# PasaLab/marlin

Hardware: AMD Instinct MI355X
Metric: dense C=AxB TFLOP/s (fp64) (higher is better)
Workload: dtype f64; 1 GPU; dgemm_20000x20000x20000_f64; m=20000, k=20000, n=20000, parallelism=single_gpu

## Files before the change

### marlin_amd/csrc/kernels.hip

```cpp

#include <hip/hip_runtime.h>
#include <stdint.h>
#include <stdlib.h>

#include <type_traits>

#include "../../include/marlin_gpu.h"
#include "gemm_group_plan.h"

typedef double v4d __attribute__((ext_vector_type(4)));
typedef float v4f __attribute__((ext_vector_type(4)));

#define DEVFN __device__ __forceinline__

DEVFN v4d mfma_16x16x4(double a, double b, v4d c) {
    return __builtin_amdgcn_mfma_f64_16x16x4f64(a, b, c, 0, 0, 0);
}
DEVFN v4f mfma_16x16x4(float a, float b, v4f c) {
    return __builtin_amdgcn_mfma_f32_16x16x4f32(a, b, c, 0, 0, 0);
}

template <typename T> struct acc_t;
template <> struct acc_t<double> { using type = v4d; };
template <> struct acc_t<float>  { using type = v4f; };

DEVFN void glds16(const void* g, void* lds) {
    __builtin_amdgcn_global_load_lds(
        (const __attribute__((address_space(1))) uint32_t*)g,
        (__attribute__((address_space(3))) uint32_t*)lds, 16, 0, 0);
}

DEVFN int32_t sload(const int32_t* p) {
    return __builtin_amdgcn_readfirstlane(*p);
}
DEVFN int64_t sload(const int64_t* p) {
    const int64_t v = *p;
    const uint32_t lo = __builtin_amdgcn_readfirstlane((uint32_t)v);
    const uint32_t hi = __builtin_amdgcn_readfirstlane((uint32_t)(v >> 32));
    return (int64_t)(((uint64_t)hi << 32) | lo);
}
DEVFN const void* sload_ptr(const void* const* p) {
    return (const void*)(uintptr_t)sload((const int64_t*)p);
}
DEVFN void* sload_ptr(void* const* p) {
    return (void*)(uintptr_t)sload((const int64_t*)p);
}

#define STAGE_FN DEVFN
#include "gemm_stage.h"

template <class S, typename T>
DEVFN void issue_pieces(const char* origin, int64_t ld, T* lds, int img,
                        int wid, int lane) {
    #pragma unroll
    for (int i = 0; i < S::PIECES; i++) {
        const stage_piece p = S::piece(wid, i, lane);
        glds16(origin + S::uni_bytes(p, ld) + S::lane_bytes(p, ld),
               &lds[img + p.lds]);
    }
}

DEVFN void block_remap(int id, int nbn, int nbm, int band, int& bm, int& bn) {
    int abands = band < 0 ? -band : band;
    int per_band = nbm * abands;
    int b0 = id / per_band;
    int w = id - b0 * per_band;
    int first_bn = b0 * abands;
    int bw = min(abands, nbn - first_bn);
    if (band < 0) {
        bn = first_bn + w / nbm;
        bm = w % nbm;
    } else {
        int sh = 8 * bw;
        int t = w / sh, l = w - t * sh;
        bm = t * 8 + l / bw;
        bn = first_bn + l % bw;
    }
}

enum { EPI_STORE = 0, EPI_TN_ADD = 1 };

template <typename T, int BETA, int BK, int BM, int WM, int WN, int PIPE,
          int TA = 0, int TB = 0, int EPI = EPI_STORE, int GRP = 0>
__launch_bounds__(WM * WN * 64, 2)
__global__ void gemm_mfma_kernel(int64_t M, int64_t N, int64_t K,
                                 const T* __restrict__ A_, int64_t lda_,
                                 const T* __restrict__ B_, int64_t ldb_,
                                 T* __restrict__ C_, int64_t ldc_,
                                 int nbm_ ,
                                 int band_ ,
                                 int phase_mask ,
                                 const T* __restrict__ addC ,
                                 const mx_group_entry* __restrict__ grp) {
    constexpr int BN = 128;
    constexpr int NWAVES = WM * WN;
    constexpr int MT = (BM / WM) / 16;
    constexpr int NT = (BN / WN) / 16;
    using ACC = typename acc_t<T>::type;
    using SA = std::conditional_t<TA != 0, stage_k<T, BM, BK, NWAVES>,
                                           stage_r<T, BM, BK, NWAVES>>;
    using SB = std::conditional_t<TB != 0, stage_r<T, BN, BK, NWAVES>,
                                           stage_k<T, BN, BK, NWAVES>>;
    constexpr int P = SA::PIECES + SB::PIECES;

    const T* __restrict__ A = A_;
    const T* __restrict__ B = B_;
    T* __restrict__ C = C_;
    int64_t lda = lda_, ldb = ldb_, ldc = ldc_;
    int nbm = nbm_, nbn = (int)(N / BN), band = band_;
    int grp_ntiles = 0;
    int id = blockIdx.x;
    if constexpr (GRP != 0) {
        static_assert(BK == 16 && BM == 128 && WM == 2 && WN == 2 &&
                      EPI == EPI_STORE, "grouped: default geometry only");
        const int count = nbm_;
        const int32_t* __restrict__ tile_start = (const int32_t*)(grp + count);
        int lo = 0, hi = count - 1;
        while (lo < hi) {
            const int mid = (lo + hi + 1) >> 1;
            if (sload(&tile_start[mid]) <= id) lo = mid; else hi = mid - 1;
        }
        const mx_group_entry* __restrict__ e = grp + lo;
        A = (const T*)sload_ptr(&e->A);
        B = (const T*)sload_ptr(&e->B);
        C = (T*)sload_ptr(&e->C);
        lda = sload(&e->lda); ldb = sload(&e->ldb); ldc = sload(&e->ldc);
        grp_ntiles = sload(&e->ntiles);
        nbm = sload(&e->nbm); nbn = sload(&e->nbn); band = sload(&e->band);
        id -= sload(&tile_start[lo]);
    }
    int bn, bm;
    block_remap(id, nbn, nbm, band, bm, bn);

    const int tid = threadIdx.x;
    const int lane = tid & 63;
    const int wid = tid >> 6;
    const int wm = wid / WN, wn = wid % WN;
    const int l15 = lane & 15, l4 = lane >> 4;

    __shared__ __align__(16) T sAB[2 * BK * BM + 2 * BN * BK];
    T* As = sAB;
    T* Bs = sAB + 2 * BK * BM;

    const int64_t row0 = (int64_t)bm * BM;
    const int64_t col0 = (int64_t)bn * BN;

    constexpr bool REGMAJOR = sizeof(T) == 8;
    const int rbase = REGMAJOR ? l4 : l4 * 4;
    constexpr int rstep = REGMAJOR ? 4 : 1;
    ACC acc[MT][NT];
    if (BETA) {
        #pragma unroll
        for (int mt = 0; mt < MT; mt++)
            #pragma unroll
            for (int nt = 0; nt < NT; nt++) {
                int64_t r = row0 + wm * (MT * 16) + mt * 16 + rbase;
                int64_t cc = col0 + wn * (NT * 16) + nt * 16 + l15;
                const T* cp = C + cc * ldc + r;
                #pragma unroll
                for (int j = 0; j < 4; j++) acc[mt][nt][j] = cp[rstep * j];
            }
    } else {
        #pragma unroll
        for (int mt = 0; mt < MT; mt++)
            #pragma unroll
            for (int nt = 0; nt < NT; nt++) acc[mt][nt] = ACC{0};
    }

    const int ntiles = GRP != 0 ? grp_ntiles : (int)(K / BK);
    const int ph = (phase_mask && (id & phase_mask)) ? (ntiles >> 1) : 0;

    auto read_quad = [&](const T* At, const T* Bt, int q, T (&a)[MT],
                         T (&b)[NT]) {
        const int kk = q * 4 + l4;
        #pragma unroll
        for (int mt = 0; mt < MT; mt++)
            a[mt] = At[SA::frag(wm * (MT * 16) + mt * 16 + l15, kk)];
        #pragma unroll
        for (int nt = 0; nt < NT; nt++)
            b[nt] = Bt[SB::frag(wn * (NT * 16) + nt * 16 + l15, kk)];
    };
    auto mfma_quad = [&](const T (&a)[MT], const T (&b)[NT]) {
        #pragma unroll
        for (int mt = 0; mt < MT; mt++)
            #pragma unroll
            for (int nt = 0; nt < NT; nt++)
                acc[mt][nt] = mfma_16x16x4(a[mt], b[nt], acc[mt][nt]);
    };

    if constexpr (!PIPE) {
    auto issue_tile = [&](int kt, int buf) {
        const int64_t kbase = (int64_t)kt * BK;
        issue_pieces<SA>((const char*)(A + SA::origin_elems(lda, row0, kbase)),
                         lda, As, buf * BK * BM, wid, lane);
        issue_pieces<SB>((const char*)(B + SB::origin_elems(ldb, col0, kbase)),
                         ldb, Bs, buf * BN * BK, wid, lane);
    };
    issue_tile(ph, 0);

    for (int s = 0; s < ntiles; s++) {
        const int buf = s & 1;
        if (s + 1 < ntiles) {
            int nxt = s + 1 + ph;
            if (nxt >= ntiles) nxt -= ntiles;
            issue_tile(nxt, buf ^ 1);
            asm volatile("s_waitcnt vmcnt(%0)" :: "n"(P) : "memory");
        } else {
            asm volatile("s_waitcnt vmcnt(0)" ::: "memory");
        }
        __builtin_amdgcn_s_barrier();

        const T* At = &As[buf * BK * BM];
        const T* Bt = &Bs[buf * BN * BK];
        #pragma unroll
        for (int q = 0; q < BK / 4; q++) {
            T a[MT], b[NT];
            read_quad(At, Bt, q, a, b);
            mfma_quad(a, b);
        }
        asm volatile("s_waitcnt lgkmcnt(0)" ::: "memory");
        __builtin_amdgcn_s_barrier();
    }
    } else {
    constexpr int Q = BK / 4;
    static_assert(Q % 2 == 0, "fragment registers ping-pong per quad");
    const int swid = __builtin_amdgcn_readfirstlane(wid);
    uint32_t a_lane[SA::PIECES], b_lane[SB::PIECES];
    int64_t a_uni[SA::PIECES], b_uni[SB::PIECES];
    int a_lds[SA::PIECES], b_lds[SB::PIECES];
    #pragma unroll
    for (int i = 0; i < SA::PIECES; i++) {
        const stage_piece p = SA::piece(swid, i, lane);
        a_lane[i] = (uint32_t)SA::lane_bytes(p, lda);
        a_uni[i] = SA::uni_bytes(p, lda);
        a_lds[i] = p.lds;
    }
    #pragma unroll
    for (int i = 0; i < SB::PIECES; i++) {
        const stage_piece p = SB::piece(swid, i, lane);
        b_lane[i] = (uint32_t)SB::lane_bytes(p, ldb);
        b_uni[i] = SB::uni_bytes(p, ldb);
        b_lds[i] = p.lds;
    }

    const char* const pA0 = (const char*)(A + SA::origin_elems(lda, row0, 0));
    const char* const pB0 = (const char*)(B + SB::origin_elems(ldb, col0, 0));
    const int64_t stepA = SA::origin_elems(lda, 0, BK) * (int64_t)sizeof(T);
    const int64_t stepB = SB::origin_elems(ldb, 0, BK) * (int64_t)sizeof(T);
    const char* pA = pA0 + ph * stepA;
    const char* pB = pB0 + ph * stepB;
    int kt = ph;
    auto issue_next = [&](int buf) {
        #pragma unroll
        for (int i = 0; i < SA::PIECES; i++)
            glds16(pA + a_uni[i] + a_lane[i], &As[buf * BK * BM + a_lds[i]]);
        #pragma unroll
        for (int i = 0; i < SB::PIECES; i++)
            glds16(pB + b_uni[i] + b_lane[i], &Bs[buf * BN * BK + b_lds[i]]);
        kt++; pA += stepA; pB += stepB;
        if (kt == ntiles) { kt = 0; pA = pA0; pB = pB0; }
    };

    T fa[2][MT], fb[2][NT];
    issue_next(0);
    if (ntiles > 1) {
        issue_next(1);
        asm volatile("s_waitcnt vmcnt(%0)" :: "n"(P) : "memory");
    } else {
        asm volatile("s_waitcnt vmcnt(0)" ::: "memory");
    }
    __builtin_amdgcn_s_barrier();
    read_quad(As, Bs, 0, fa[0], fb[0]);

    auto step = [&](int s, auto ahead) {
        constexpr int AHEAD = decltype(ahead)::value;
        const int buf = s & 1;
        const T* At = &As[buf * BK * BM];
        const T* Bt = &Bs[buf * BN * BK];
        #pragma unroll
        for (int q = 0; q + 1 < Q; q++) {
            read_quad(At, Bt, q + 1, fa[(q + 1) & 1], fb[(q + 1) & 1]);
            mfma_quad(fa[q & 1], fb[q & 1]);
        }
        __builtin_amdgcn_sched_barrier(0);
        asm volatile("s_waitcnt lgkmcnt(0)" ::: "memory");
        if constexpr (AHEAD >= 1) {
            asm volatile("s_waitcnt vmcnt(0)" ::: "memory");
            __builtin_amdgcn_s_barrier();
            __builtin_amdgcn_sched_barrier(0);
            read_quad(&As[(buf ^ 1) * BK * BM], &Bs[(buf ^ 1) * BN * BK], 0,
                      fa[0], fb[0]);
            if constexpr (AHEAD >= 2) issue_next(buf);
        }
        mfma_quad(fa[1], fb[1]);
        if constexpr (AHEAD >= 1) {
            #pragma unroll
            for (int g = 0; g < MT + NT; g++) {
                __builtin_amdgcn_sched_group_barrier(0x008, 1, 0);
                __builtin_amdgcn_sched_group_barrier(0x100, 1, 0);
            }
            if constexpr (AHEAD >= 2) {
                #pragma unroll
                for (int g = 0; g < P; g++) {
                    __builtin_amdgcn_sched_group_barrier(0x008, 1, 0);
                    __builtin_amdgcn_sched_group_barrier(0x010, 1, 0);
                }
            }
        }
        __builtin_amdgcn_sched_barrier(0);
    };
    int s = 0;
    for (; s + 2 < ntiles; s++) step(s, std::integral_constant<int, 2>{});
    if (s + 1 < ntiles) { step(s, std::integral_constant<int, 1>{}); s++; }
    step(s, std::integral_constant<int, 0>{});
    }

    if constexpr (EPI == EPI_TN_ADD) {
        static_assert(std::is_same<T, float>::value && !BETA && !PIPE &&
                      BM == 128 && WM == 2 && WN == 2,
                      "fused epilogue: fp32 default geometry, two-barrier loop");
        static_assert(64 * BN == 2 * BK * BM + 2 * BN * BK,
                      "the 64x128 stage fills the k-loop buffers exactly");
        float* stage = sAB;
        v4f* stage4 = (v4f*)sAB;
        #pragma unroll
        for (int half = 0; half < 2; half++) {
            __builtin_amdgcn_s_barrier();
            if (wm == half) {
                #pragma unroll
                for (int mt = 0; mt < 4; mt++)
                    #pragma unroll
                    for (int nt = 0; nt < 4; nt++) {
                        int rloc = mt * 16 + l4 * 4;
                        int cc = wn * 64 + nt * 16 + l15;
                        #pragma unroll
                        for (int j = 0; j < 4; j++)
                            stage[(rloc + j) * BN + cc] = acc[mt][nt][j];
                    }
            }
            __builtin_amdgcn_s_barrier();
            #pragma unroll
            for (int i = 0; i < 8; i++) {
                int idx = tid + i * 256;
                int rloc = idx >> 5;
                int q = idx & 31;
                int64_t r = row0 + half * 64 + rloc;
                int64_t off = col0 + 4 * q + r * ldc;
                v4f v = stage4[rloc * (BN / 4) + q];
                if (addC) {
                    const v4f* ap = (const v4f*)(addC + off);
                    v4f av = *ap;
                    v.x += av.x; v.y += av.y; v.z += av.z; v.w += av.w;
                }
                *(v4f*)(C + off) = v;
            }
        }
    } else {
    #pragma unroll
    for (int mt = 0; mt < MT; mt++)
        #pragma unroll
        for (int nt = 0; nt < NT; nt++) {
            int64_t r = row0 + wm * (MT * 16) + mt * 16 + rbase;
            int64_t cc = col0 + wn * (NT * 16) + nt * 16 + l15;
            T* cp = C + cc * ldc + r;
            #pragma unroll
            for (int j = 0; j < 4; j++) cp[rstep * j] = acc[mt][nt][j];
        }
    }
}


__device__ __forceinline__ uint64_t splitmix64(uint64_t z) {
    z = (z ^ (z >> 30)) * 0xBF58476D1CE4E5B9ULL;
    z = (z ^ (z >> 27)) * 0x94D049BB133111EBULL;
    return z ^ (z >> 31);
}

template <typename T>
__global__ void fill_random_kernel(T* __restrict__ buf, int64_t m, int64_t n,
                                   int64_t ld, uint64_t seed) {
    int64_t i = (int64_t)blockIdx.x * blockDim.x + threadIdx.x;
    int64_t total = m * n;
    int64_t stride = (int64_t)gridDim.x * blockDim.x;
    for (; i < total; i += stride) {
        int64_t c = i / m, r = i - c * m;
        uint64_t z = splitmix64(seed + (uint64_t)(i + 1) * 0x9E3779B97F4A7C15ULL);
        buf[c * ld + r] = (T)((double)(z >> 11) * (1.0 / 9007199254740992.0));
    }
}

template <typename T>
__global__ void zero_pad_kernel(T* __restrict__ buf, int64_t rows_total,
                                int64_t cols_total, int64_t ld,
                                int64_t m, int64_t n) {
    int64_t i = (int64_t)blockIdx.x * blockDim.x + threadIdx.x;
    int64_t total = rows_total * cols_total;
    int64_t stride = (int64_t)gridDim.x * blockDim.x;
    for (; i < total; i += stride) {
        int64_t c = i / rows_total, r = i - c * rows_total;
        if (r >= m || c >= n) buf[c * ld + r] = (T)0;
    }
}


template <typename T>
__global__ void map_kernel(int op, int64_t n, const T* __restrict__ a,
                           const T* __restrict__ b, double scalar,
                           T* __restrict__ c) {
    const T s = (T)scalar;
    int64_t i = (int64_t)blockIdx.x * blockDim.x + threadIdx.x;
    int64_t stride = (int64_t)gridDim.x * blockDim.x;
    for (; i < n; i += stride) {
        T x = a[i];
        T y;
        switch (op) {
            case MX_OP_ADD:   y = x + b[i]; break;
            case MX_OP_SUB:   y = x - b[i]; break;
            case MX_OP_EMUL:  y = x * b[i]; break;
            case MX_OP_ADDS:  y = x + s; break;
            case MX_OP_SUBS:  y = x - s; break;
            case MX_OP_RSUBS: y = s - x; break;
            case MX_OP_MULS:  y = x * s; break;
            case MX_OP_DIVS:  y = x / s; break;
            default:          y = s / x; break;
        }
        c[i] = y;
    }
}

template <typename T>
__global__ void sum_stage1_kernel(int64_t n, const T* __restrict__ a,
                                  double* __restrict__ partials) {
    __shared__ double sm[256];
    double acc = 0;
    int64_t i = (int64_t)blockIdx.x * blockDim.x + threadIdx.x;
    int64_t stride = (int64_t)gridDim.x * blockDim.x;
    for (; i < n; i += stride) acc += (double)a[i];
    sm[threadIdx.x] = acc;
    __syncthreads();
    for (int w = 128; w > 0; w >>= 1) {
        if (threadIdx.x < w) sm[threadIdx.x] += sm[threadIdx.x + w];
        __syncthreads();
    }
    if (threadIdx.x == 0) partials[blockIdx.x] = sm[0];
}

__global__ void sum_stage2_kernel(int nparts, const double* __restrict__ p,
                                  double* __restrict__ out) {
    __shared__ double sm[256];
    double acc = 0;
    for (int i = threadIdx.x; i < nparts; i += 256) acc += p[i];
    sm[threadIdx.x] = acc;
    __syncthreads();
    for (int w = 128; w > 0; w >>= 1) {
        if (threadIdx.x < w) sm[threadIdx.x] += sm[threadIdx.x + w];
        __syncthreads();
    }
    if (threadIdx.x == 0) *out = sm[0];
}

template <typename T>
__global__ void transpose_kernel(int64_t m, int64_t n,
                                 const T* __restrict__ in,
                                 T* __restrict__ out) {
    __shared__ T tile[32][33];
    int64_t tm = (m + 31) / 32;
    int64_t bi = blockIdx.x % tm;
    int64_t bj = blockIdx.x / tm;
    int tx = threadIdx.x % 32, ty = threadIdx.x / 32;
    int64_t r0 = bi * 32, c0 = bj * 32;
    #pragma unroll
    for (int k = 0; k < 4; k++) {
        int64_t r = r0 + tx, c = c0 + ty + k * 8;
        if (r < m && c < n) tile[ty + k * 8][tx] = in[c * m + r];
    }
    __syncthreads();
    #pragma unroll
    for (int k = 0; k < 4; k++) {
        int64_t r = c0 + tx, c = r0 + ty + k * 8;
        if (r < n && c < m) out[c * n + r] = tile[tx][ty + k * 8];
    }
}

template <typename T>
__global__ void gemv_partial_kernel(int64_t m, int64_t n, int64_t lda,
                                    const T* __restrict__ A,
                                    const T* __restrict__ x,
                                    double* __restrict__ partial,
                                    int nchunks) {
    int64_t nrb = (m + 255) / 256;
    int64_t rb = blockIdx.x % nrb;
    int chunk = (int)(blockIdx.x / nrb);
    int64_t r = rb * 256 + threadIdx.x;
    int64_t clen = (n + nchunks - 1) / nchunks;
    int64_t c0 = chunk * clen;
    int64_t c1 = c0 + clen < n ? c0 + clen : n;
    if (r >= m) return;
    double a0 = 0, a1 = 0, a2 = 0, a3 = 0;
    int64_t j = c0;
    for (; j + 4 <= c1; j += 4) {
        a0 += (double)A[(j + 0) * lda + r] * (double)x[j + 0];
        a1 += (double)A[(j + 1) * lda + r] * (double)x[j + 1];
        a2 += (double)A[(j + 2) * lda + r] * (double)x[j + 2];
        a3 += (double)A[(j + 3) * lda + r] * (double)x[j + 3];
    }
    for (; j < c1; j++)
        a0 += (double)A[j * lda + r] * (double)x[j];
    partial[(int64_t)chunk * m + r] = ((a0 + a1) + (a2 + a3));
}

template <typename T>
__global__ void gemv_reduce_kernel(int64_t m, int nchunks,
                                   const double* __restrict__ partial,
                                   T* __restrict__ y) {
    int64_t r = (int64_t)blockIdx.x * blockDim.x + threadIdx.x;
    if (r >= m) return;
    double acc = 0;
    for (int c = 0; c < nchunks; c++) acc += partial[(int64_t)c * m + r];
    y[r] = (T)acc;
}

static mx_gemm_cfg_t g_last_gemm_cfg = {};
static int g_last_gemm_loop = 0;
static int g_last_gemm_op[2] = {0, 0};

struct gemm_call {
    int64_t M, N, K;
    const void* A; int64_t lda;
    const void* B; int64_t ldb;
    void* C; int64_t ldc;
    int band, phase_mask;
    int loopsel;
    bool pitch32;
    hipStream_t stream;
};

template <typename T, int BETA, int BK, int BM, int WM, int WN,
          int TA = 0, int TB = 0>
static void launch_gemm(const gemm_call& g) {
    const bool pipe = g.pitch32 && (g.loopsel >= 0 ? g.loopsel == 1
                                    : !(sizeof(T) == 4 && BK == 16));
    g_last_gemm_cfg = mx_gemm_cfg_t{sizeof(T) == 4, BETA, BK, BM, WM * WN,
                                    g.band, g.phase_mask};
    g_last_gemm_loop = pipe ? 1 : 0;
    g_last_gemm_op[0] = TA;
    g_last_gemm_op[1] = TB;
    auto go = [&](auto pipe_c) {
        hipLaunchKernelGGL(
            (gemm_mfma_kernel<T, BETA, BK, BM, WM, WN, decltype(pipe_c)::value,
                              TA, TB>),
            dim3((unsigned)((g.M / BM) * (g.N / 128))), dim3(WM * WN * 64),
            0, g.stream, g.M, g.N, g.K, (const T*)g.A, g.lda,
            (const T*)g.B, g.ldb, (T*)g.C, g.ldc, (int)(g.M / BM), g.band,
            g.phase_mask, (const T*)nullptr,
            (const mx_group_entry*)nullptr);
    };
    if (pipe) go(std::integral_constant<int, 1>{});
    else      go(std::integral_constant<int, 0>{});
}

static int g_last_gemm_group_problems = 0;
static int64_t g_last_gemm_group_blocks = 0;

template <typename T, int BETA, int TA, int TB>
static void launch_gemm_grouped(int count, unsigned blocks, int band0,
                                const mx_group_entry* table, int loopsel,
                                bool pitch32, hipStream_t stream) {
    const bool pipe = pitch32 && (loopsel >= 0 ? loopsel == 1
                                  : sizeof(T) != 4);
    g_last_gemm_cfg = mx_gemm_cfg_t{sizeof(T) == 4, BETA, 16, 128, 4, band0, 0};
    g_last_gemm_loop = pipe ? 1 : 0;
    g_last_gemm_op[0] = TA;
    g_last_gemm_op[1] = TB;
    g_last_gemm_group_problems = count;
    g_last_gemm_group_blocks = blocks;
    auto go = [&](auto pipe_c) {
        hipLaunchKernelGGL(
            (gemm_mfma_kernel<T, BETA, 16, 128, 2, 2, decltype(pipe_c)::value,
                              TA, TB, EPI_STORE, 1>),
            dim3(blocks), dim3(256), 0, stream, (int64_t)0, (int64_t)0,
            (int64_t)0, (const T*)nullptr, (int64_t)0, (const T*)nullptr,
            (int64_t)0, (T*)nullptr, (int64_t)0, count, 0, 0,
            (const T*)nullptr, table);
    };
    if (pipe) go(std::integral_constant<int, 1>{});
    else      go(std::integral_constant<int, 0>{});
}

extern "C" {

void mxk_gemm_remap_knobs(int* band_width, int* plain_bands) {
    static const char* bandenv = getenv("MARLIN_GEMM_BAND");
    static const char* remap = getenv("MARLIN_GEMM_REMAP");
    int bandw = bandenv ? atoi(bandenv) : 8;
    *band_width = bandw < 1 ? 8 : bandw;
    *plain_bands = remap && remap[0] == 'b';
}

void mxk_last_gemm_group(int* problems, int64_t* blocks) {
    *problems = g_last_gemm_group_problems;
    *blocks = g_last_gemm_group_blocks;
}

int mxk_gemm_grouped(int is_fp32, int beta_one, int trans_a, int trans_b,
                     const mx_group_plan* plan, void* ws, hipStream_t stream) {
    const int count = (int)plan->entries.size();
    if (count == 0) return 0;
    const size_t eb = (size_t)count * sizeof(mx_group_entry);
    if (hipMemcpyAsync(ws, plan->entries.data(), eb, hipMemcpyHostToDevice,
                       stream) != hipSuccess ||
        hipMemcpyAsync((char*)ws + eb, plan->tile_start.data(),
                       (size_t)(count + 1) * sizeof(int32_t),
                       hipMemcpyHostToDevice, stream) != hipSuccess)
        return -2;
    static const char* loopenv = getenv("MARLIN_GEMM_LOOP");
    const int loopsel = !loopenv ? -1 : loopenv[0] == 't' ? 0
                      : loopenv[0] == 'p' ? 1 : -1;
    const unsigned blocks = (unsigned)plan->blocks();
    const int band0 = plan->entries[0].band;
    const mx_group_entry* table = (const mx_group_entry*)ws;
    auto form = [&](auto t, auto beta) {
        using T = decltype(t);
        constexpr int BT = decltype(beta)::value;
        auto l = [&](auto ta, auto tb) {
            launch_gemm_grouped<T, BT, decltype(ta)::value,
                                decltype(tb)::value>(
                count, blocks, band0, table, loopsel, plan->pitch32, stream);
        };
        using one = std::integral_constant<int, 1>;
        using zero = std::integral_constant<int, 0>;
        if (trans_a && trans_b) l(one{}, one{});
        else if (trans_a)       l(one{}, zero{});
        else if (trans_b)       l(zero{}, one{});
        else                    l(zero{}, zero{});
    };
    using one = std::integral_constant<int, 1>;
    using zero = std::integral_constant<int, 0>;
    if (is_fp32) { if (beta_one) form(float{}, one{}); else form(float{}, zero{}); }
    else         { if (beta_one) form(double{}, one{}); else form(double{}, zero{}); }
    return (int)hipGetLastError() == 0 ? 0 : -2;
}

void mxk_last_gemm_config(mx_gemm_cfg_t* out) { *out = g_last_gemm_cfg; }

void mxk_last_gemm_loop(int* out) { *out = g_last_gemm_loop; }

static inline bool pitch_ok(int64_t ld, int64_t rows, int64_t elems16) {
    return ld >= rows && ld % elems16 == 0;
}

void mxk_last_gemm_op(int* trans_a, int* trans_b) {
    *trans_a = g_last_gemm_op[0];
    *trans_b = g_last_gemm_op[1];
}

int mxk_gemm_op(int is_fp32, int beta_one, int trans_a, int trans_b,
                int64_t M, int64_t N, int64_t K,
                const void* A, int64_t lda, const void* B, int64_t ldb,
                void* C, int64_t ldc, hipStream_t stream) {
    if ((trans_a | trans_b) & ~1) return -4;
    if (M < 0 || N < 0 || K < 0) return -4;
    if (M == 0 || N == 0) return 0;
    {
        const int64_t e16 = is_fp32 ? 4 : 2;
        if (!pitch_ok(lda, trans_a ? K : M, e16) ||
            !pitch_ok(ldb, trans_b ? N : K, e16) ||
            !pitch_ok(ldc, M, e16))
            return -4;
    }
    if (K == 0) {
        if (!beta_one) {
            size_t es = is_fp32 ? 4 : 8;
            hipError_t e = hipMemset2DAsync(C, (size_t)ldc * es, 0,
                                            (size_t)M * es, (size_t)N, stream);
            if (e != hipSuccess) return -2;
        }
        return 0;
    }
    if (M % 128 || N % 128 || K % 16) return -4;
    int nbn = (int)(N / 128);
    static const char* bandenv = getenv("MARLIN_GEMM_BAND");
    int bandw = bandenv ? atoi(bandenv) : 8;
    if (bandw < 1) bandw = 8;
    int band = nbn < bandw ? nbn : bandw;
    static const char* remap = getenv("MARLIN_GEMM_REMAP");
    if (remap && remap[0] == 'b') band = -band;
    static const char* cfg = getenv("MARLIN_GEMM_CFG");
    bool bk32 = (K % 32 == 0) && cfg && cfg[0] == 'b' && cfg[1] == 'k';
    bool bm256 = (M % 256 == 0) && !is_fp32 && cfg && cfg[0] == 'b' && cfg[1] == 'm';
    if (trans_a || trans_b) bk32 = bm256 = false;
    static const char* phenv = getenv("MARLIN_GEMM_PHASE");
    int phase_mask = phenv ? atoi(phenv) : 0;
    static const char* loopenv = getenv("MARLIN_GEMM_LOOP");
    const int loopsel = !loopenv ? -1 : loopenv[0] == 't' ? 0
                      : loopenv[0] == 'p' ? 1 : -1;
    const bool pitch32 = lda < ((int64_t)1 << 26) && ldb < ((int64_t)1 << 26);
    const gemm_call g{M, N, K, A, lda, B, ldb, C, ldc, band, phase_mask,
                      loopsel, pitch32, stream};
    auto dispatch = [&](auto t, auto beta) {
        using T = decltype(t);
        constexpr int BT = decltype(beta)::value;
        if (trans_a && trans_b) launch_gemm<T, BT, 16, 128, 2, 2, 1, 1>(g);
        else if (trans_a)       launch_gemm<T, BT, 16, 128, 2, 2, 1, 0>(g);
        else if (trans_b)       launch_gemm<T, BT, 16, 128, 2, 2, 0, 1>(g);
        else if (bm256) {
            if constexpr (sizeof(T) == 8) launch_gemm<T, BT, 16, 256, 4, 2>(g);
        }
        else if (bk32)          launch_gemm<T, BT, 32, 128, 2, 4>(g);
        else                    launch_gemm<T, BT, 16, 128, 2, 2>(g);
    };
    using one = std::integral_constant<int, 1>;
    using zero = std::integral_constant<int, 0>;
    if (is_fp32) { if (beta_one) dispatch(float{}, one{}); else dispatch(float{}, zero{}); }
    else         { if (beta_one) dispatch(double{}, one{}); else dispatch(double{}, zero{}); }
    return (int)hipGetLastError() == 0 ? 0 : -2;
}

int mxk_gemm(int is_fp32, int beta_one,
             int64_t M, int64_t N, int64_t K,
             const void* A, int64_t lda, const void* B, int64_t ldb,
             void* C, int64_t ldc, hipStream_t stream) {
    return mxk_gemm_op(is_fp32, beta_one, 0, 0, M, N, K, A, lda, B, ldb, C,
                       ldc, stream);
}

int mxk_sgemm_tn_epilogue(int64_t M, int64_t N, int64_t K,
                          const float* A, int64_t lda,
                          const float* B, int64_t ldb,
                          float* C, int64_t ldc, const float* addC,
                          hipStream_t stream) {
    if (M <= 0 || N <= 0 || K <= 0) return -4;
    if (M % 128 || N % 128 || K % 16) return -4;
    if (!pitch_ok(lda, M, 4) || !pitch_ok(ldb, K, 4) || !pitch_ok(ldc, N, 4))
        return -4;
    int nbm = (int)(M / 128), nbn = (int)(N / 128);
    int band = nbn < 8 ? nbn : 8;
    dim3 grid((unsigned)(nbm * nbn)), block(256);
    hipLaunchKernelGGL(
        (gemm_mfma_kernel<float, 0, 16, 128, 2, 2, 0, 0, 0, EPI_TN_ADD>),
        grid, block, 0, stream, M, N, K, A, lda, B, ldb, C, ldc, nbm, band,
        0, addC, (const mx_group_entry*)nullptr);
    return (int)hipGetLastError() == 0 ? 0 : -2;
}

int mxk_fill_random(int is_fp32, void* buf, int64_t m, int64_t n, int64_t ld,
                    uint64_t seed, hipStream_t stream) {
    dim3 grid(2048), block(256);
    if (is_fp32)
        hipLaunchKernelGGL(fill_random_kernel<float>, grid, block, 0, stream,
                           (float*)buf, m, n, ld, seed);
    else
        hipLaunchKernelGGL(fill_random_kernel<double>, grid, block, 0, stream,
                           (double*)buf, m, n, ld, seed);
    return (int)hipGetLastError() == 0 ? 0 : -2;
}

int mxk_zero_pad(int is_fp32, void* buf, int64_t rows_total, int64_t cols_total,
                 int64_t ld, int64_t m, int64_t n, hipStream_t stream) {
    dim3 grid(2048), block(256);
    if (is_fp32)
        hipLaunchKernelGGL(zero_pad_kernel<float>, grid, block, 0, stream,
                           (float*)buf, rows_total, cols_total, ld, m, n);
    else
        hipLaunchKernelGGL(zero_pad_kernel<double>, grid, block, 0, stream,
                           (double*)buf, rows_total, cols_total, ld, m, n);
    return (int)hipGetLastError() == 0 ? 0 : -2;
}

int mxk_map(int is_fp32, int op, int64_t n, const void* a, const void* b,
            double scalar, void* c, hipStream_t stream) {
    dim3 grid(2048), block(256);
    if (is_fp32)
        hipLaunchKernelGGL(map_kernel<float>, grid, block, 0, stream, op, n,
                           (const float*)a, (const float*)b, scalar, (float*)c);
    else
        hipLaunchKernelGGL(map_kernel<double>, grid, block, 0, stream, op, n,
                           (const double*)a, (const double*)b, scalar,
                           (double*)c);
    return (int)hipGetLastError() == 0 ? 0 : -2;
}

int mxk_sum(int is_fp32, int64_t n, const void* a, double* partials,
            double* out, hipStream_t stream) {
    dim3 grid(1024), block(256);
    if (is_fp32)
        hipLaunchKernelGGL(sum_stage1_kernel<float>, grid, block, 0, stream,
                           n, (const float*)a, partials);
    else
        hipLaunchKernelGGL(sum_stage1_kernel<double>, grid, block, 0, stream,
                           n, (const double*)a, partials);
    hipLaunchKernelGGL(sum_stage2_kernel, dim3(1), block, 0, stream, 1024,
                       partials, out);
    return (int)hipGetLastError() == 0 ? 0 : -2;
}

int mxk_transpose(int is_fp32, int64_t m, int64_t n, const void* in,
                  void* out, hipStream_t stream) {
    int64_t tm = (m + 31) / 32, tn = (n + 31) / 32;
    dim3 grid((unsigned)(tm * tn)), block(256);
    if (is_fp32)
        hipLaunchKernelGGL(transpose_kernel<float>, grid, block, 0, stream,
                           m, n, (const float*)in, (float*)out);
    else
        hipLaunchKernelGGL(transpose_kernel<double>, grid, block, 0, stream,
                           m, n, (const double*)in, (double*)out);
    return (int)hipGetLastError() == 0 ? 0 : -2;
}

int mxk_gemv(int is_fp32, int64_t m, int64_t n, int64_t lda, const void* A,
             const void* x, double* partial, void* y, hipStream_t stream) {
    int64_t nrb = (m + 255) / 256;
    int nchunks = 32;
    dim3 grid((unsigned)(nrb * nchunks)), block(256);
    if (is_fp32) {
        hipLaunchKernelGGL(gemv_partial_kernel<float>, grid, block, 0, stream,
                           m, n, lda, (const float*)A, (const float*)x,
                           partial, nchunks);
        hipLaunchKernelGGL(gemv_reduce_kernel<float>, dim3((unsigned)nrb),
                           block, 0, stream, m, nchunks, partial, (float*)y);
    } else {
        hipLaunchKernelGGL(gemv_partial_kernel<double>, grid, block, 0, stream,
                           m, n, lda, (const double*)A, (const double*)x,
                           partial, nchunks);
        hipLaunchKernelGGL(gemv_reduce_kernel<double>, dim3((unsigned)nrb),
                           block, 0, stream, m, nchunks, partial, (double*)y);
    }
    return (int)hipGetLastError() == 0 ? 0 : -2;
}

}
```

### tools_dev/cmp_gemm_asm.py

```python
#!/usr/bin/env python3
import re
import subprocess
import sys

CLASSES = (("mfma", r"v_mfma_"), ("lds_rd", r"ds_read"),
           ("dma", r"global_load_lds"), ("barrier", r"s_barrier"),
           ("waitcnt", r"s_waitcnt"))


def key_of(demangled):
    m = re.match(r"void gemm_mfma_kernel<([^>]*)>", demangled)
    if m:
        a = [x.strip() for x in m.group(1).split(",")]
        a = [re.sub(r"^\(\w+\)", "", x) for x in a]
        a += ["0"] * (11 - len(a))
        return tuple(a)
    if demangled.startswith("sgemm_mfma_tn_epilogue_kernel"):
        return ("float", "0", "16", "128", "2", "2", "0", "0", "0", "1", "0")
    return None


def kernels(path):
    text = open(path).read()
    names = re.findall(r"^\s*\.amdhsa_kernel (\S+)", text, re.M)
    dem = subprocess.run(["c++filt"], input="\n".join(names), text=True,
                         capture_output=True, check=True).stdout.split("\n")
    out = {}
    for name, d in zip(names, dem):
        k = key_of(d)
        if k is None:
            continue
        res = text.split("\n" + name + ":", 1)[1]
        body = res.split("\n", 1)[1].split(".Lfunc_end", 1)[0]
        ins = []
        for line in body.split("\n"):
            line = line.split(";")[0].strip()
            if not line or line.startswith("."):
                if re.match(r"\.LBB\d+_\d+:", line):
                    ins.append(re.sub(r"\.LBB\d+_", ".LBB_", line))
                continue
            ins.append(re.sub(r"\.LBB\d+_", ".LBB_", line))
        meta = text.split(".amdhsa_kernel " + name + "\n", 1)[1]
        meta = meta.split(".end_amdhsa_kernel", 1)[0]

        def note(tag):
            return re.search(r"; " + tag + r": (\d+)", res).group(1)
        out[k] = dict(
            ins=ins, n=sum(1 for i in ins if not i.endswith(":")),
            vgpr=note("TotalNumVgprs"), sgpr=note("TotalNumSgprs"),
            scratch=note("ScratchSize"), occ=note("Occupancy"),
            lds=re.search(r"\.amdhsa_group_segment_fixed_size (\d+)",
                          meta).group(1),
            loop=loop_counts(ins))
    return out


def loop_counts(ins):
    pos = {l[:-1]: i for i, l in enumerate(ins) if l.endswith(":")}
    br = {}
    for i, l in enumerate(ins):
        m = re.match(r"s_c?branch\w* (\.LBB_\d+)", l)
        if m and m.group(1) in pos:
            br[i] = pos[m.group(1)]
    best = None
    for i, j in br.items():
        if j >= i:
            continue
        lo, hi, grown = j, i, True
        while grown:
            grown = False
            for q, p in br.items():
                if lo <= q <= hi and p < lo:
                    lo, grown = p, True
                if q > hi and lo <= p <= hi and any(
                        lo <= q2 <= hi and hi < p2 <= q
                        for q2, p2 in br.items()):
                    hi, grown = q, True
        c = tuple(sum(1 for x in ins[lo:hi] if re.match(rx, x))
                  for _, rx in CLASSES)
        if best is None or (c[0], hi - lo) > (best[0][0], best[1]):
            best = (c, hi - lo)
    return best[0] if best else (0,) * len(CLASSES)


def main():
    old, new = kernels(sys.argv[1]), kernels(sys.argv[2])
    assert set(old) <= set(new), set(old) - set(new)
    added = sorted(set(new) - set(old))
    print("| kernel <T,BETA,BK,BM,WM,WN,PIPE,TA,TB,EPI,GRP> | instr old/new | "
          "identical | VGPR | SGPR | scratch | LDS | occ | loop "
          + "/".join(n for n, _ in CLASSES) + " |")
    print("|---|---|---|---|---|---|---|---|---|")
    bad = 0
    for k in sorted(old):
        o, n = old[k], new[k]
        same = o["ins"] == n["ins"]

        def pair(f):
            return o[f] if o[f] == n[f] else f"{o[f]}->{n[f]}"
        loop = "/".join(map(str, n["loop"]))
        if o["loop"] != n["loop"]:
            loop = "/".join(map(str, o["loop"])) + " -> " + loop
        if (int(n["scratch"]) > int(o["scratch"]) or
                int(n["occ"]) < int(o["occ"]) or
                [o["loop"][i] for i in (0, 2, 3)] !=
                [n["loop"][i] for i in (0, 2, 3)]):
            bad += 1
            loop += " **FAIL**"
        print(f"| {','.join(k)} | {o['n']}/{n['n']} | "
              f"{'yes' if same else 'no'} | {pair('vgpr')} | {pair('sgpr')} | "
              f"{pair('scratch')} | {pair('lds')} | {pair('occ')} | {loop} |")
    for k in added:
        n, t = new[k], new.get(k[:-1] + ("0",))
        loop = "/".join(map(str, n["loop"]))
        twin = "no twin"
        if t:
            twin = ("twin loop equal" if t["loop"] == n["loop"] else
                    "twin loop " + "/".join(map(str, t["loop"])))
            twin += f", twin instr {t['n']} VGPR {t['vgpr']} SGPR {t['sgpr']}"
        print(f"| {','.join(k)} | new/{n['n']} | new | {n['vgpr']} | "
              f"{n['sgpr']} | {n['scratch']} | {n['lds']} | {n['occ']} | "
              f"{loop} ({twin}) |")
    ident = sum(old[k]["ins"] == new[k]["ins"] for k in old)
    print(f"\n{len(old)} kernels, {ident} identical, {len(added)} new, "
          f"{bad} failing a "
          "condition (scratch up, occupancy down, loop MFMA/DMA/barrier "
          "counts changed)")
    return 1 if bad else 0


if __name__ == "__main__":
    sys.exit(main())
```

Baseline: 70.49 TFLOP/s.

## Interleave LDS fragment reads with MFMAs per quad and unroll k-loop by two

Adds sched_group_barrier patterns inside each quad so ds_reads for the next fragment are spread between MFMAs, leaving a tail of MFMAs to hide LDS latency. The loop-end read group is also batched per wave count. The main k-loop is unrolled by two with compile-time buffer indices, removing the s&1 address arithmetic. This trades larger code and more rigid scheduling for better overlap of LDS reads with matrix math.

```diff
diff --git a/marlin_amd/csrc/kernels.hip b/marlin_amd/csrc/kernels.hip
--- a/marlin_amd/csrc/kernels.hip
+++ b/marlin_amd/csrc/kernels.hip
@@ -224,6 +224,15 @@
     } else {
     constexpr int Q = BK / 4;
     static_assert(Q % 2 == 0, "fragment registers ping-pong per quad");
+    constexpr int RD_TAIL = 4;
+    static_assert(MT * NT > RD_TAIL, "a quad needs MFMAs ahead of its tail");
+    constexpr int RD_PER = (MT + NT + MT * NT - RD_TAIL - 1) / (MT * NT - RD_TAIL);
+    constexpr int RD_GROUPS = (MT + NT + RD_PER - 1) / RD_PER;
+    constexpr int RD_LEAD =
+        sizeof(T) == 4 ? (MT * NT - RD_GROUPS - RD_TAIL) / 2 : 0;
+    constexpr int LQ_PER = NWAVES == 8 ? 2 : 1;
+    constexpr int LQ_GROUPS = (MT + NT + LQ_PER - 1) / LQ_PER;
+    constexpr bool UNROLL2 = !(sizeof(T) == 4 && BETA && BK == 16);
     const int swid = __builtin_amdgcn_readfirstlane(wid);
     uint32_t a_lane[SA::PIECES], b_lane[SB::PIECES];
     int64_t a_uni[SA::PIECES], b_uni[SB::PIECES];
@@ -272,17 +281,26 @@
     __builtin_amdgcn_s_barrier();
     read_quad(As, Bs, 0, fa[0], fb[0]);
 
-    auto step = [&](int s, auto ahead) {
+    auto step = [&](auto bufc, auto ahead) {
         constexpr int AHEAD = decltype(ahead)::value;
-        const int buf = s & 1;
+        const int buf = bufc;
         const T* At = &As[buf * BK * BM];
         const T* Bt = &Bs[buf * BN * BK];
         #pragma unroll
         for (int q = 0; q + 1 < Q; q++) {
             read_quad(At, Bt, q + 1, fa[(q + 1) & 1], fb[(q + 1) & 1]);
             mfma_quad(fa[q & 1], fb[q & 1]);
-        }
-        __builtin_amdgcn_sched_barrier(0);
+            if constexpr (RD_LEAD > 0)
+                __builtin_amdgcn_sched_group_barrier(0x008, RD_LEAD, 0);
+            #pragma unroll
+            for (int g = 0; g < RD_GROUPS; g++) {
+                __builtin_amdgcn_sched_group_barrier(0x008, 1, 0);
+                __builtin_amdgcn_sched_group_barrier(0x100, RD_PER, 0);
+            }
+            __builtin_amdgcn_sched_group_barrier(
+                0x008, MT * NT - RD_LEAD - RD_GROUPS, 0);
+            __builtin_amdgcn_sched_barrier(0);
+        }
         asm volatile("s_waitcnt lgkmcnt(0)" ::: "memory");
         if constexpr (AHEAD >= 1) {
             asm volatile("s_waitcnt vmcnt(0)" ::: "memory");
@@ -295,9 +313,9 @@
         mfma_quad(fa[1], fb[1]);
         if constexpr (AHEAD >= 1) {
             #pragma unroll
-            for (int g = 0; g < MT + NT; g++) {
+            for (int g = 0; g < LQ_GROUPS; g++) {
                 __builtin_amdgcn_sched_group_barrier(0x008, 1, 0);
-                __builtin_amdgcn_sched_group_barrier(0x100, 1, 0);
+                __builtin_amdgcn_sched_group_barrier(0x100, LQ_PER, 0);
             }
             if constexpr (AHEAD >= 2) {
                 #pragma unroll
@@ -309,10 +327,17 @@
         }
         __builtin_amdgcn_sched_barrier(0);
     };
+    using std::integral_constant;
     int s = 0;
-    for (; s + 2 < ntiles; s++) step(s, std::integral_constant<int, 2>{});
-    if (s + 1 < ntiles) { step(s, std::integral_constant<int, 1>{}); s++; }
-    step(s, std::integral_constant<int, 0>{});
+    if constexpr (UNROLL2) {
+        for (; s + 3 < ntiles; s += 2) {
+            step(integral_constant<int, 0>{}, integral_constant<int, 2>{});
+            step(integral_constant<int, 1>{}, integral_constant<int, 2>{});
+        }
+    }
+    for (; s + 2 < ntiles; s++) step(s & 1, integral_constant<int, 2>{});
+    if (s + 1 < ntiles) { step(s & 1, integral_constant<int, 1>{}); s++; }
+    step(s & 1, integral_constant<int, 0>{});
     }
 
     if constexpr (EPI == EPI_TN_ADD) {
diff --git a/tools_dev/cmp_gemm_asm.py b/tools_dev/cmp_gemm_asm.py
--- a/tools_dev/cmp_gemm_asm.py
+++ b/tools_dev/cmp_gemm_asm.py
@@ -101,10 +101,12 @@
         loop = "/".join(map(str, n["loop"]))
         if o["loop"] != n["loop"]:
             loop = "/".join(map(str, o["loop"])) + " -> " + loop
+        def per_step(c):
+            steps = max(1, c[0] // 64)
+            return [c[i] / steps for i in (0, 2, 3)]
         if (int(n["scratch"]) > int(o["scratch"]) or
                 int(n["occ"]) < int(o["occ"]) or
-                [o["loop"][i] for i in (0, 2, 3)] !=
-                [n["loop"][i] for i in (0, 2, 3)]):
+                per_step(o["loop"]) != per_step(n["loop"])):
             bad += 1
             loop += " **FAIL**"
         print(f"| {','.join(k)} | {o['n']}/{n['n']} | "
diff --git a/tools_dev/gemm_loop_waits.py b/tools_dev/gemm_loop_waits.py
--- /dev/null
+++ b/tools_dev/gemm_loop_waits.py
@@ -0,0 +1,171 @@
+#!/usr/bin/env python3
+import os
+import re
+import subprocess
+import sys
+import tempfile
+
+HERE = os.path.dirname(os.path.abspath(__file__))
+KERNELS_HIP = os.path.join(os.path.dirname(HERE), "marlin_amd", "csrc",
+                           "kernels.hip")
+FIELDS = ("T", "BETA", "BK", "BM", "WM", "WN", "PIPE", "TA", "TB", "EPI",
+          "GRP")
+
+
+def compile_listing(src=KERNELS_HIP, out=None):
+    if out is None:
+        out = os.path.join(tempfile.mkdtemp(prefix="gemm_asm_"), "kernels.s")
+    subprocess.run(["hipcc", "--offload-arch=gfx950", "-O3", "-std=c++17",
+                    "--cuda-device-only", "-S", src, "-o", out], check=True,
+                   capture_output=True)
+    return out
+
+
+def key_of(demangled):
+    m = re.match(r"void gemm_mfma_kernel<([^>]*)>", demangled)
+    if not m:
+        return None
+    a = [re.sub(r"^\(\w+\)", "", x.strip()) for x in m.group(1).split(",")]
+    return tuple(a + ["0"] * (len(FIELDS) - len(a)))
+
+
+def _instructions(body):
+    ins = []
+    for line in body.split("\n"):
+        line = line.split(";")[0].strip()
+        if re.match(r"\.LBB\d+_\d+:", line):
+            ins.append(line)
+        elif line and not line.startswith("."):
+            ins.append(line)
+    return ins
+
+
+def loop_body(ins):
+    pos = {l[:-1]: i for i, l in enumerate(ins) if l.endswith(":")}
+    spans = []
+    for i, l in enumerate(ins):
+        m = re.match(r"s_c?branch\w* (\.LBB\d+_\d+)", l)
+        if not m or pos.get(m.group(1), i) >= i:
+            continue
+        lo = pos[m.group(1)]
+        n = sum(1 for x in ins[lo:i + 1] if x.startswith("v_mfma_"))
+        if n:
+            spans.append((lo, i, n))
+    inner = [s for s in spans
+             if not any(t != s and s[0] <= t[0] and t[1] <= s[1]
+                        for t in spans)]
+    if not inner:
+        return []
+    lo, hi, _ = max(inner, key=lambda s: s[2])
+    return ins[lo:hi + 1]
+
+
+def classify(op):
+    if op.startswith("v_mfma_"):
+        return "mfma"
+    if op.startswith("ds_read"):
+        return "ds_read"
+    if op.startswith("global_load_lds") or (
+            op.startswith(("global_load", "buffer_load")) and " lds" in op):
+        return "dma"
+    if op.startswith("s_barrier"):
+        return "barrier"
+    if op.startswith("s_waitcnt"):
+        return "waitcnt"
+    if op.startswith("v_"):
+        return "valu"
+    if op.startswith("s_") and not op.startswith(("s_nop", "s_cbranch",
+                                                  "s_branch")):
+        return "salu"
+    return "other"
+
+
+def lgkm_waits(body):
+    out = []
+    pending = []
+    mfmas = 0
+    seen_barrier = False
+    for rnd in (0, 1):
+        for l in body:
+            c = classify(l)
+            if c == "mfma":
+                mfmas += 1
+            elif c == "ds_read":
+                pending.append(mfmas)
+            elif c == "barrier":
+                seen_barrier = True
+            elif c == "waitcnt":
+                m = re.search(r"lgkmcnt\((\d+)\)", l)
+                if not m:
+                    continue
+                keep = min(int(m.group(1)), len(pending))
+                n = int(m.group(1))
+                forced = pending[:len(pending) - keep]
+                dist = mfmas - forced[-1] if forced else None
+                pending = pending[len(pending) - keep:]
+                if rnd:
+                    top = bool(forced) and seen_barrier
+                    out.append((n, dist, top))
+                if forced:
+                    seen_barrier = False
+    return out
+
+
+def kernels(path):
+    text = open(path).read()
+    names = re.findall(r"^\s*\.amdhsa_kernel (\S+)", text, re.M)
+    dem = subprocess.run(["c++filt"], input="\n".join(names), text=True,
+                         capture_output=True, check=True).stdout.split("\n")
+    out = {}
+    for name, d in zip(names, dem):
+        k = key_of(d)
+        if k is None:
+            continue
+        res = text.split("\n" + name + ":", 1)[1]
+        ins = _instructions(res.split("\n", 1)[1].split(".Lfunc_end", 1)[0])
+        meta = text.split(".amdhsa_kernel " + name + "\n", 1)[1]
+        meta = meta.split(".end_amdhsa_kernel", 1)[0]
+
+        def note(tag):
+            return int(re.search(r"; " + tag + r": (\d+)", res).group(1))
+        body = loop_body(ins)
+        counts = {}
+        for l in body:
+            c = classify(l)
+            counts[c] = counts.get(c, 0) + 1
+        out[k] = dict(
+            key=dict(zip(FIELDS, k)), counts=counts, waits=lgkm_waits(body),
+            vgpr=note("TotalNumVgprs"), sgpr=note("TotalNumSgprs"),
+            scratch=note("ScratchSize"), occ=note("Occupancy"),
+            lds=int(re.search(r"\.amdhsa_group_segment_fixed_size (\d+)",
+                              meta).group(1)))
+    return out
+
+
+def waits_text(waits):
+    return " ".join(f"({n}):{'-' if d is None else d}{'^' if top else ''}"
+                    for n, d, top in waits)
+
+
+def main():
+    args = sys.argv[1:]
+    if args and args[0] == "--compile":
+        path = compile_listing(*(args[1:2] or [KERNELS_HIP]))
+    else:
+        path = args[0]
+    ks = kernels(path)
+    cols = ("mfma", "valu", "salu", "ds_read", "dma", "barrier", "waitcnt")
+    print("| kernel <" + ",".join(FIELDS) + "> | " + " | ".join(cols) +
+          " | VGPR | scratch | LDS | occ | lgkmcnt waits (n):MFMAs since "
+          "the youngest forced read, ^ = loop-top wait |")
+    print("|---" * (len(cols) + 6) + "|")
+    for k in sorted(ks):
+        r = ks[k]
+        print(f"| {','.join(k)} | " +
+              " | ".join(str(r["counts"].get(c, 0)) for c in cols) +
+              f" | {r['vgpr']} | {r['scratch']} | {r['lds']} | {r['occ']} | "
+              f"{waits_text(r['waits'])} |")
+
+
+if __name__ == "__main__":
+    main()
```

New measurement: 73.68 TFLOP/s (median of 6 runs). 1.05x the previous value.
